# duckdb-faiss-ext/duckdb-faiss-ext

Hardware: AMD Instinct MI355X
Metric: queries/sec, FlatL2 d=128 N=10000000 nq=10000 k=10 (higher is better)
Workload: dtype f32 results (bf16 matrix-pipe coarse filter with a proven bound + exact f32 re-scoring of the candidates); 1 GPU; Flat L2 d=128 N=10000000 nq=10000 k=10; queries_per_call=10000, replicas=1, exchange=none

## Files before the change

duckdb-faiss-ext_amd/csrc/flat_collect.hip:

```cpp
#include "flat_collect.h"

#include <algorithm>
#include <climits>
#include <cmath>
#include <cstring>
#include <type_traits>

#include <rocprim/device/device_radix_sort.hpp>
#include <rocprim/device/device_segmented_radix_sort.hpp>

namespace mvs {

__global__ __launch_bounds__(256) void collect_colsum_kernel(const float *__restrict__ src, long long nrows, int dp,
                                                            int interleaved, float *__restrict__ sum) {
	const int g8 = dp / 8, rl = threadIdx.x / g8, c8 = threadIdx.x % g8, nrl = 256 / g8;
	float acc[8] = {0.f, 0.f, 0.f, 0.f, 0.f, 0.f, 0.f, 0.f};
	const long long r0 = (long long)blockIdx.x * 1024;
	__shared__ float red[256 * 8];
	const bool idle = rl >= nrl;
	for (long long r = r0 + rl; !idle && r < r0 + 1024 && r < nrows; r += nrl) {
		const float4 s0 = *(const float4 *)(src + (size_t)r * dp + c8 * 8);
		const float4 s1 = *(const float4 *)(src + (size_t)r * dp + c8 * 8 + 4);
		float v[8];
		if (!interleaved) {
// ... 470 lines not shown
				}
			}
		}
		part[which][r] = acc;
	}
	__syncthreads();
	if (tid < 64) {
		const long long q = q0 + tid;
		if (q < nq) {
			const float xn = part[0][tid], xnc = part[1][tid], mun = part[2][tid], dq2 = part[3][tid];
			qn[q] = xn;
			const float yn = __uint_as_float(max_norm_bits[2]), ync = __uint_as_float(max_norm_bits[8]);
			const float dyc = __uint_as_float(I8 ? i8_bits[0] : max_norm_bits[12]);
			const double u = 5.9604644775390625e-08, infl = 1.0001;
			const double S = sqrt((double)xn * infl) * sqrt((double)yn * infl);
			const double Sc = sqrt((double)xnc * infl) * sqrt((double)ync * infl);
			const double MY = sqrt((double)mun * infl) * sqrt((double)yn * infl);
			const double al = IS_L2 ? 2.0 : 1.0;
			const double bmax = IS_L2 ? (double)ync : MY;
			const double rnd_worst = al * (0.0078125 + 1.52587890625e-05) * Sc;
			const double ndq = sqrt((double)dq2 * infl), ndy = sqrt((double)dyc * infl);
			const double rnd_actual = ndq * sqrt((double)ync * infl) + (al * sqrt((double)xnc * infl) + ndq) * ndy;
			const double rnd = I8 ? rnd_actual
			                      : (bound_mode == 0 ? rnd_worst : (rnd_actual < rnd_worst || !(rnd_actual == rnd_actual) ? rnd_actual : rnd_worst));
			const double es = I8 ? rnd + 0.5 * (double)i8_unit
			                     : rnd + 1.25 * ((double)d / 16.0) * CL_MFMA_UNITS * u * ((1.0 + 0.0079) * al * Sc + bmax);
			double E;
			if (IS_L2)
				E = es + 4.0 * u * ((double)xnc + ync) + (double)d * u * ync + 2.0 * d * u * S + 4.0 * u * ((double)xn + yn) +
				    2.0 * ((double)d + 8.0) * u * ((double)xn + yn);
			else
				E = es + 4.0 * u * Sc + 2.0 * u * MY + (double)d * u * MY + (double)d * u * S;
			float r = (float)(2.0 * E * (1.0 + 0.0009765625) + 8.0 * u * (Sc + MY + (double)xnc + ync) + 1e-30);
			const bool ok = isfinite(xn) && isfinite(yn) && isfinite(ync) && isfinite(mun) && isfinite(dq2) && isfinite(dyc) && isfinite(r) && r < 1e30f;
			if (!ok) {
				r = __uint_as_float(0x7fc00000u);
				fail_q[atomicAdd(fail_cnt, 1)] = (int)q;
			}
			e2[q] = r;
		} else if (q < nq_e2) {
			e2[q] = __uint_as_float(0x7fc00000u);
		}
	}
	const float alpha = IS_L2 ? 2.0f : 1.0f;
	if (I8) {
		i32x4n *qf8 = (i32x4n *)qf;
		for (int i = tid; i < 4 * 2 * 64; i += 256) {
			const int lane = i & 63, kb = (i >> 6) & 1, qb = i >> 7;
			const int r = qb * 16 + (lane & 15);
			if (q0 + qb * 16 >= nq_frag)
				continue;
			i32x4n w = {0, 0, 0, 0};
#pragma unroll
			for (int e = 0; e < 16; ++e) {
				const int kk = kb * 64 + 16 * (lane >> 4) + e;
				const int qv = (q0 + r < nq && kk < d) ? cl_i8_q(alpha * (xs[r][kk] - ms[kk]), inv_sa) : 0;
				w[e >> 2] |= (int)((unsigned)(qv & 255) << (8 * (e & 3)));
			}
			qf8[((q0 / 16 + qb) * 2 + kb) * 64 + lane] = w;
		}
	}
	for (int i = tid; i < 4 * 4 * 64 && !I8; i += 256) {
		const int lane = i & 63, kb = (i >> 6) & 3, qb = i >> 8;
		const int r = qb * 16 + (lane & 15);
		if (q0 + qb * 16 >= nq_frag)
			continue;
		bf16x8 hi;
#pragma unroll
		for (int e = 0; e < 8; ++e) {
			const int kk = kb * 32 + 8 * (lane >> 4) + e;
			hi[e] = (__bf16)((q0 + r < nq && kk < d) ? alpha * (xs[r][kk] - ms[kk]) : 0.f);
		}
		qf[((q0 / 16 + qb) * 4 + kb) * 64 + lane] = hi;
	}
	const unsigned neutral = ~f2key(-FLT_MAX);
	for (int i = tid; i < 64 * stride; i += 256) {
		const long long q = q0 + i / stride;
		if (q < nq)
			gslot[q * stride + (i % stride)] = neutral;
	}
	if (tid < 64 && q0 + tid < nq) {
		ctl_seg[q0 + tid] = 0;
		ctl_seg[nq + q0 + tid] = 0;
	}
	if (blockIdx.x == 0 && tid < 64)
		ctl_hdr[tid] = 0;
}
void launch_collect_query_prep(int metric, const float *d_x, int64_t nq, int d, const float *d_mu, const unsigned *d_max_norm_bits,
                               void *d_qf, float *d_qn, float *d_e2, int *d_fail_cnt, int *d_fail_q, unsigned *d_gslot, int stride,
                               int *d_ctl_hdr, int *d_ctl_seg, hipStream_t st, const unsigned *d_i8_bits, float i8_sa, float i8_unit) {
	if (nq <= 0)
		return;
	const long long nq_frag = (nq + CL_QBLOCK - 1) / CL_QBLOCK * CL_QBLOCK, nq_e2 = (nq + 255) / 256 * 256;
	const dim3 grid((unsigned)(nq_frag / 64));
	const bool i8 = i8_unit > 0.f;
	auto kern = metric == METRIC_L2 ? (i8 ? collect_query_prep_kernel<true, true> : collect_query_prep_kernel<true>)
	                                : (i8 ? collect_query_prep_kernel<false, true> : collect_query_prep_kernel<false>);
	hipLaunchKernelGGL(kern, grid, dim3(256), 0, st, d_x, (long long)nq, d, d_mu, d_max_norm_bits, (bf16x8 *)d_qf, nq_frag, d_qn, d_e2, nq_e2,
	                   d_fail_cnt, d_fail_q, tune().cl_bound_mode, d_gslot, stride, d_ctl_hdr, d_ctl_seg, d_i8_bits, i8_sa, i8_unit);
	MVS_HIP(hipGetLastError());
}

typedef float f32x4acc __attribute__((ext_vector_type(4)));
template <int KCH, bool IS_L2, bool COLLECT, bool SEL = false, int NC = 16, bool I8 = false>
__global__ __launch_bounds__(256, I8 ? 3 : 2) void flat_bf16_collect_kernel(const CollectArgs a) {
	constexpr int DP = KCH * 16;
	constexpr int KB = I8 ? DP / 64 : DP / 32;
	constexpr int PITCH = I8 ? DP : DP * 2;
	constexpr int C = PITCH / 16;
	constexpr int TILE_BYTES = CL_BN * PITCH;
	constexpr int SUB = cl_sub(I8);
	constexpr int STAGE_ROWS = SUB * CL_BN;
	constexpr int STAGE_BYTES = SUB * TILE_BYTES;
	constexpr int NDMA = STAGE_BYTES / 1024;
	constexpr int DMA_PER_WAVE = NDMA / 4;
	constexpr int QCAP = cl_qcap(I8);
	static_assert(C == (I8 ? 8 : 16) && KB == (I8 ? 2 : 4) && NDMA % 4 == 0 && STAGE_ROWS % 64 == 0, "d = 128 geometry");
	typedef typename std::conditional<I8, i32x4n, bf16x8>::type frag_t;
	typedef typename std::conditional<I8, i32x4n, f32x4acc>::type acc_t;
	typedef typename std::conditional<I8, i32x2n, f32x2n>::type bnd_t;
	typedef typename std::conditional<I8, int, float>::type val_t;
	const float unit = a.i8_unit;

	extern __shared__ __attribute__((aligned(16))) float smem[];
	char *tbuf = (char *)smem;
	float *nbuf = (float *)(tbuf + 2 * STAGE_BYTES);
	unsigned long long *qbuf = (unsigned long long *)(nbuf + 2 * STAGE_ROWS);
	float *cqtab = (float *)(qbuf + QCAP);
	unsigned *qctl = (unsigned *)(cqtab + CL_QBLOCK);
	float *qval = (float *)(qctl + 16);
	float *cqstage = qval + QCAP;

	const int tid = threadIdx.x, lane = tid & 63;
	const int wave = __builtin_amdgcn_readfirstlane(tid >> 6);
	const int hq = lane >> 4, c = lane & 15;
	int split, qb;
	if (a.xcd_map) {
		const int xcd = blockIdx.x & 7, idx = blockIdx.x >> 3;
		split = (idx / a.nqb) * 8 + xcd;
		qb = idx % a.nqb;
	} else {
		split = blockIdx.x / a.nqb;
		qb = blockIdx.x % a.nqb;
	}
	const long long r_begin = a.row_first + (long long)split * a.split_rows;
	long long r_end = r_begin + a.split_rows;
	if (r_end > a.n)
		r_end = a.n;
	const int ntiles = r_end > r_begin ? (int)((r_end - r_begin + STAGE_ROWS - 1) / STAGE_ROWS) : 0;
	if (tid == 0)
		qctl[7] = 0u;

	const int qw = qb * CL_QBLOCK + wave * 128;

	frag_t bq[8][KB];
	{
		const frag_t *qsrc = (const frag_t *)a.qf;
#pragma unroll
		for (int cb = 0; cb < 8; ++cb) {
			const size_t qblk16 = (size_t)qb * (CL_QBLOCK / 16) + wave * 8 + cb;
#pragma unroll
			for (int kb = 0; kb < KB; ++kb)
				bq[cb][kb] = qsrc[(qblk16 * KB + kb) * 64 + lane];
		}
	}

	unsigned dma_off;
	{
		const int rr = I8 ? 8 * wave + (lane >> 3) : 4 * wave + (lane >> 4);
		dma_off = (unsigned)(rr * PITCH + (((lane & (C - 1)) ^ (rr & (C - 1))) * 16));
	}
	auto dma_issue = [&](int u, int i) {
		const char *base = (const char *)a.yb + (size_t)(r_begin + (long long)u * STAGE_ROWS) * PITCH + (size_t)i * 4096;
		__builtin_amdgcn_global_load_lds((glb_f32c *)(base + dma_off),
		                                 (lds_f32c *)(smem + ((u & 1) * STAGE_BYTES + (i * 4 + wave) * 1024) / 4), 16, 0, 0);
	};
	auto dma_norms = [&](int u) {
		const float *base = a.yn + (r_begin + (long long)u * STAGE_ROWS);
#pragma unroll
		for (int j = 0; j < STAGE_ROWS / 64; ++j)
			__builtin_amdgcn_global_load_lds((glb_f32c *)(base + 64 * j + lane),
			                                 (lds_f32c *)(smem + (2 * STAGE_BYTES) / 4 + (u & 1) * STAGE_ROWS + 64 * j), 4, 0, 0);
	};
	const bool use_tab = a.pbnd != nullptr;
	const bool frozen = use_tab && (a.flags & CL_FROZEN) != 0;
	constexpr int tab_shift = I8 ? 1 : 2;
	constexpr int duty_mask = (!COLLECT ? 3 : (NC > 32 ? 255 : 63)) >> (I8 ? 1 : 0);
	const int duty_phase = split * 13 + 5;
	bool tab_pending = false;
	const float inv_unit = I8 ? 1.0f / unit : 0.f;
	auto dma_bounds = [&]() {
		const float *base = a.pbnd + (size_t)qb * CL_QBLOCK + wave * 128;
		float *dst = (I8 ? cqstage : cqtab) + wave * 128;
		__builtin_amdgcn_global_load_lds((glb_f32c *)(base + lane), (lds_f32c *)dst, 4, 0, 16 );
		__builtin_amdgcn_global_load_lds((glb_f32c *)(base + 64 + lane), (lds_f32c *)(dst + 64), 4, 0, 16);
		tab_pending = I8;
	};
	auto tab_cvt = [&]() {
		if (!I8 || !tab_pending)
			return;
		tab_pending = false;
		const float p0 = cqstage[wave * 128 + lane], p1 = cqstage[wave * 128 + 64 + lane];
		((int *)cqtab)[wave * 128 + lane] = cl_i8_thr(p0, inv_unit);
		((int *)cqtab)[wave * 128 + 64 + lane] = cl_i8_thr(p1, inv_unit);
	};
	if (ntiles > 0) {
#pragma unroll
		for (int i = 0; i < DMA_PER_WAVE; ++i)
			dma_issue(0, i);
		dma_norms(0);
		if (use_tab)
			dma_bounds();
	}
	__syncthreads();
	tab_cvt();

	const unsigned rbase = (unsigned)(c * PITCH) | (unsigned)(((hq ^ c) & (C - 1)) * 16);
	constexpr int WQCAP = QCAP / 4;
	const unsigned qcnt_lds = (unsigned)(uintptr_t)((__attribute__((address_space(3))) unsigned *)qctl);
	const unsigned qbuf_lds = (unsigned)(uintptr_t)((__attribute__((address_space(3))) unsigned long long *)qbuf) + (unsigned)(wave * WQCAP * 8);
	const unsigned qval_lds = (unsigned)(uintptr_t)((__attribute__((address_space(3))) float *)qval) + (unsigned)(wave * WQCAP * 4);
	const unsigned cq_lds = (unsigned)(uintptr_t)((__attribute__((address_space(3))) float *)cqtab) + (unsigned)((wave * 64 + c) * 8);

	int ovf = 0;
	int wfill = 0, wpub = 0;
	auto publish = [&]() __attribute__((always_inline)) {
		const unsigned n = (unsigned)wfill < (unsigned)WQCAP ? (unsigned)wfill : (unsigned)WQCAP;
		for (unsigned e = (unsigned)wpub + lane; e < n && !frozen; e += 64) {
			unsigned long long ent;
			float v;
			asm volatile("ds_read_b64 %0, %2\n\tds_read_b32 %1, %3\n\ts_waitcnt lgkmcnt(0)"
			             : "=&v"(ent), "=&v"(v)
			             : "v"(qbuf_lds + 8u * e), "v"(qval_lds + 4u * e)
			             : "memory");
			const unsigned row = (unsigned)ent;
			typedef __attribute__((address_space(1))) unsigned *GU;
			__hip_atomic_fetch_min((GU)(a.gslot + (size_t)(unsigned)(ent >> 32) * NC) + (row & (unsigned)(NC - 1)), skey(v), __ATOMIC_RELAXED,
			                       __HIP_MEMORY_SCOPE_AGENT);
		}
		wpub = (int)n;
	};
	auto wdrain = [&]() __attribute__((always_inline)) {
		publish();
		const unsigned n = (unsigned)wpub;
		wfill = 0;
		wpub = 0;
		if (!COLLECT || n == 0u)
			return;
		unsigned long long base = 0ull;
		if (lane == 0) {
			const unsigned long long n64 = n;
			typedef __attribute__((address_space(1))) unsigned long long *GUL;
			asm volatile("global_atomic_add_x2 %0, %1, %2, off sc0\n\ts_waitcnt vmcnt(0)"
			             : "=&v"(base)
			             : "v"((GUL)a.stream_cnt), "v"(n64)
			             : "memory");
		}
		const unsigned blo = (unsigned)__builtin_amdgcn_readfirstlane((int)(unsigned)base);
		const unsigned bhi = (unsigned)__builtin_amdgcn_readfirstlane((int)(unsigned)(base >> 32));
		base = ((unsigned long long)bhi << 32) | blo;
		for (unsigned e = lane; e < n; e += 64) {
			unsigned long long ent;
			float v;
			asm volatile("ds_read_b64 %0, %2\n\tds_read_b32 %1, %3\n\ts_waitcnt lgkmcnt(0)"
			             : "=&v"(ent), "=&v"(v)
			             : "v"(qbuf_lds + 8u * e), "v"(qval_lds + 4u * e)
			             : "memory");
			if ((long long)(base + e) < a.stream_cap) {
				typedef __attribute__((address_space(1))) unsigned long long *GUL;
				*((GUL)a.stream + (base + e)) = ent;
				if (a.stream_s)
					a.stream_s[base + e] = v;
			}
		}
		ovf |= (long long)(base + n) >= a.stream_cap ? 1 : 0;
	};
	auto rare = [&](const acc_t (&sv)[2], int rb, int t, bool any_t, bnd_t cqv, long long row0, int nvalid, unsigned rowbits) {
		if (__builtin_expect(__builtin_amdgcn_ballot_w64(any_t) == 0ull, 1))
			return;
		int qo = qw;
		MVS_OPAQUE_VGPR(qo);
		unsigned m0 = 0u, m1 = 0u;
		if (any_t) {
#pragma unroll
			for (int r = 0; r < 4; ++r) {
				const bool in = 16 * rb + 4 * hq + r < nvalid;
				m0 |= (in && sv[0][r] >= cqv[0]) ? 1u << r : 0u;
				m1 |= (in && sv[1][r] >= cqv[1]) ? 1u << r : 0u;
			}
			if (SEL) {
				const unsigned rbits = (rowbits >> (16 * rb + 4 * hq)) & 15u;
				m0 &= rbits;
				m1 &= rbits;
			}
		}
		unsigned m = m0 | (m1 << 4);
		while (__builtin_amdgcn_ballot_w64(m != 0u) != 0ull) {
			const bool has = m != 0u;
			const int j8 = has ? __builtin_ctz(m) : 0;
			m &= m - 1u;
			const int i = j8 >> 2, j = j8 & 3;
			const val_t s0 = i ? sv[1][0] : sv[0][0], s1 = i ? sv[1][1] : sv[0][1], s2 = i ? sv[1][2] : sv[0][2], s3 = i ? sv[1][3] : sv[0][3];
			const val_t lo = (j & 1) ? s1 : s0;
			const val_t hi = (j & 1) ? s3 : s2;
			const float v = I8 ? (float)((j & 2) ? hi : lo) * unit : (float)((j & 2) ? hi : lo);
			const unsigned row = (unsigned)(row0 + 16 * rb + 4 * hq + j);
			const unsigned q = (unsigned)(qo + 32 * t + 16 * i + c);
			if (!(COLLECT && ovf) && __builtin_expect(wfill + (int)__builtin_popcountll(__builtin_amdgcn_ballot_w64(has)) > WQCAP, 0))
				wdrain();
			const bool counting = COLLECT && ovf;
			const unsigned long long act = __builtin_amdgcn_ballot_w64(has && !counting);
			const unsigned pos = (unsigned)wfill + __builtin_amdgcn_mbcnt_hi((unsigned)(act >> 32), __builtin_amdgcn_mbcnt_lo((unsigned)act, 0u));
			wfill = __builtin_amdgcn_readfirstlane(wfill + (int)__builtin_popcountll(act));
			if (has) {
				const unsigned long long ent = ((unsigned long long)q << 32) | row;
				if (__builtin_expect(!counting, 1)) {
					asm volatile("ds_write_b64 %0, %1\n\tds_write_b32 %2, %3" ::"v"(qbuf_lds + 8u * pos), "v"(ent), "v"(qval_lds + 4u * pos), "v"(v) : "memory");
				} else {
					typedef __attribute__((address_space(1))) unsigned *GU;
					__hip_atomic_fetch_min((GU)(a.gslot + (size_t)q * NC) + (row & (unsigned)(NC - 1)), skey(v), __ATOMIC_RELAXED,
					                       __HIP_MEMORY_SCOPE_AGENT);
					const unsigned one = 1u;
					asm volatile("ds_add_u32 %0, %1" ::"v"(qcnt_lds + 28u), "v"(one) : "memory");
				}
			}
		}
	};

	for (int u = 0; u < ntiles; ++u) {
		const int period = u < 4 ? 1 : (u < 32 ? 8 : (u < 256 ? 32 : 128));
		const bool full = !frozen && (use_tab ? ((u + duty_phase) & duty_mask) == 0 : (u % period) == 0);
		if (use_tab && !full && u > 0 && (u & ((1 << tab_shift) - 1)) == 0)
			dma_bounds();
		if (full) {
			publish();
			int qo = qw;
			MVS_OPAQUE_VGPR(qo);
			f32x2n v = {0.f, 0.f};
#pragma unroll 1
			for (int i = 0; i < 2; ++i) {
				const int q = qo + 32 * hq + 16 * i + c;
				const int qc = q < a.nq ? q : 0;
				const float e2v = __builtin_nontemporal_load(a.e2 + qc);
				constexpr int SUBN = NC > 32 ? 32 : NC, NSUB = NC / SUBN;
				const int rank = NSUB == 1 ? a.nclass - 1 : (a.nclass + NSUB - 1) / NSUB - 1;
				unsigned kth = 0u;
#pragma unroll 1
				for (int sb = 0; sb < NSUB; ++sb) {
				const unsigned long long *src = (const unsigned long long *)(a.gslot + (size_t)qc * NC + sb * SUBN);
				unsigned long long w[SUBN / 2];
#pragma unroll
				for (int j = 0; j < SUBN / 2; ++j)
					w[j] = __hip_atomic_load(src + j, __ATOMIC_RELAXED, __HIP_MEMORY_SCOPE_AGENT);
#pragma unroll
				for (int j = 0; j < SUBN / 2; ++j)
					asm volatile("" : "+v"(w[j]));
				unsigned key[SUBN];
#pragma unroll
				for (int j = 0; j < SUBN / 2; ++j) {
					key[2 * j] = (unsigned)w[j];
					key[2 * j + 1] = (unsigned)(w[j] >> 32);
				}
#pragma unroll
				for (int kbit = 2; kbit <= SUBN; kbit <<= 1)
#pragma unroll
					for (int jb = kbit >> 1; jb > 0; jb >>= 1)
#pragma unroll
						for (int x0 = 0; x0 < SUBN; ++x0) {
							const int x1 = x0 ^ jb;
							if (x1 > x0) {
								const unsigned lo = key[x0] < key[x1] ? key[x0] : key[x1];
								const unsigned hi = key[x0] < key[x1] ? key[x1] : key[x0];
								const bool asc = (x0 & kbit) == 0;
								key[x0] = asc ? lo : hi;
								key[x1] = asc ? hi : lo;
							}
						}
				unsigned ks = key[0];
#pragma unroll
				for (int j = 1; j < SUBN; ++j)
					ks = (rank == j) ? key[j] : ks;
				kth = ks > kth ? ks : kth;
				}
				const unsigned neutral = skey(-FLT_MAX);
				const float B = skey2f(kth < neutral ? kth : neutral);
				const float bv = q < a.nq ? B - e2v : __uint_as_float(0x7fc00000u);
				v[0] = i == 0 ? bv : v[0];
				v[1] = i == 1 ? bv : v[1];
			}
			if (I8) {
				const i32x2n vi = {cl_i8_thr(v[0], inv_unit), cl_i8_thr(v[1], inv_unit)};
				*(i32x2n *)(cqtab + (wave * 64 + hq * 16 + c) * 2) = vi;
			} else {
				*(f32x2n *)(cqtab + (wave * 64 + hq * 16 + c) * 2) = v;
			}
			if (use_tab) {
				unsigned long long bits;
				__builtin_memcpy(&bits, &v, 8);
				__hip_atomic_store((unsigned long long *)(a.pbnd + (size_t)qb * CL_QBLOCK + (wave * 64 + hq * 16 + c) * 2), bits, __ATOMIC_RELAXED,
				                   __HIP_MEMORY_SCOPE_AGENT);
			}
		}
#pragma unroll 1
		for (int sub = 0; sub < SUB; ++sub) {
		frag_t A[KB][2];
		acc_t Y[2];
		{
			const unsigned nb_lds = (unsigned)(uintptr_t)((lds_f32c *)(nbuf + (u & 1) * STAGE_ROWS + sub * CL_BN + 4 * hq));
			asm volatile("ds_read_b128 %0, %2\n\tds_read_b128 %1, %2 offset:64" : "=&v"(Y[0]), "=&v"(Y[1]) : "v"(nb_lds) : "memory");
			const unsigned ab =
			    (unsigned)(uintptr_t)((lds_f32c *)(smem + ((u & 1) * STAGE_BYTES + sub * TILE_BYTES) / 4)) + rbase;
#pragma unroll
			for (int kb = 0; kb < KB; ++kb) {
				asm volatile("ds_read_b128 %0, %1" : "=v"(A[kb][0]) : "v"(ab ^ (unsigned)(kb * 64)) : "memory");
				if (I8)
					asm volatile("ds_read_b128 %0, %1 offset:2048" : "=v"(A[kb][1]) : "v"(ab ^ (unsigned)(kb * 64)) : "memory");
				else
					asm volatile("ds_read_b128 %0, %1 offset:4096" : "=v"(A[kb][1]) : "v"(ab ^ (unsigned)(kb * 64)) : "memory");
			}
		}
		if (sub == 0) {
#pragma unroll
			for (int i = 0; i < DMA_PER_WAVE; ++i)
				dma_issue(u + 1, i);
			dma_norms(u + 1);
		}
		const long long row0 = r_begin + ((long long)u * SUB + sub) * CL_BN;
		const int nvalid = (int)((r_end - row0) < CL_BN ? (r_end - row0) : CL_BN);
		unsigned rowbits = 0xFFFFFFFFu;
		if (SEL) {
			typedef __attribute__((address_space(4))) const unsigned cuint;
			rowbits = *((cuint *)a.rowmask + (row0 >> 5));
		}

		acc_t acc[2][2];
		bnd_t cqv[2];
		const val_t lowest = I8 ? (val_t)INT_MIN : (val_t)-INFINITY;
		val_t mx0 = lowest, mx1 = lowest;
		auto vmax = [](val_t x, val_t y) {
			if constexpr (I8)
				return x > y ? x : y;
			else
				return __builtin_fmaxf(x, y);
		};
		auto fold = [&](acc_t &p, int rb, int i) {
			(void)rb;
			if (i == 0)
				mx0 = vmax(vmax(vmax(vmax(mx0, p[0]), p[1]), p[2]), p[3]);
			else
				mx1 = vmax(vmax(vmax(vmax(mx1, p[0]), p[1]), p[2]), p[3]);
		};
		auto any_of = [&](bnd_t cqp) {
			const bool r = (mx0 >= cqp[0]) || (mx1 >= cqp[1]);
			mx0 = lowest;
			mx1 = lowest;
			return r;
		};
#pragma unroll
		for (int t = 0; t < 4; ++t) {
			asm volatile("ds_read_b64 %0, %1" : "=v"(cqv[t & 1]) : "v"(cq_lds + (unsigned)(t * 128)) : "memory");
#pragma unroll
			for (int rb = 0; rb < 2; ++rb) {
				const int prb = rb ^ 1, pt = rb == 0 ? t - 1 : t;
#pragma unroll
				for (int kb = 0; kb < KB; ++kb) {
					if constexpr (I8) {
						if (t == 0) {
							if (rb == 0 && kb == 0)
								asm volatile("s_waitcnt lgkmcnt(4)" : "+v"(A[0][0]), "+v"(Y[0]), "+v"(Y[1]));
							else if (rb == 0 && kb == 1)
								asm volatile("s_waitcnt lgkmcnt(2)" : "+v"(A[1][0]));
							else if (rb == 1 && kb == 0)
								asm volatile("s_waitcnt lgkmcnt(0)" : "+v"(A[0][1]), "+v"(A[1][1]), "+v"(cqv[0]));
						}
					} else if (t == 0) {
						if (rb == 0 && kb == 0)
							asm volatile("s_waitcnt lgkmcnt(8)" : "+v"(A[0][0]), "+v"(Y[0]), "+v"(Y[1]));
						else if (rb == 0 && kb == 1)
							asm volatile("s_waitcnt lgkmcnt(6)" : "+v"(A[1][0]));
						else if (rb == 0 && kb == 2)
							asm volatile("s_waitcnt lgkmcnt(4)" : "+v"(A[2][0]));
						else if (rb == 0 && kb == 3)
							asm volatile("s_waitcnt lgkmcnt(2)" : "+v"(A[3][0]));
						else if (rb == 1 && kb == 0)
							asm volatile("s_waitcnt lgkmcnt(0)" : "+v"(A[0][1]), "+v"(A[1][1]), "+v"(A[2][1]), "+v"(A[3][1]), "+v"(cqv[0]));
					}
#pragma unroll
					for (int i = 0; i < 2; ++i) {
						if constexpr (I8)
							acc[rb][i] = __builtin_amdgcn_mfma_i32_16x16x64_i8(A[kb][rb], bq[2 * t + i][kb], kb == 0 ? Y[rb] : acc[rb][i], 0, 0, 0);
						else if (kb == 0)
							acc[rb][i] = __builtin_amdgcn_mfma_f32_16x16x32_bf16(A[kb][rb], bq[2 * t + i][kb], Y[rb], 0, 0, 0);
						else
							acc[rb][i] = __builtin_amdgcn_mfma_f32_16x16x32_bf16(A[kb][rb], bq[2 * t + i][kb], acc[rb][i], 0, 0, 0);
					}
					if (pt >= 0 && kb < 2)
						fold(acc[prb][kb], prb, kb);
					__builtin_amdgcn_sched_barrier(0);
				}
				if (pt >= 0) {
					if (rb == 0)
						asm volatile("s_waitcnt lgkmcnt(0)" : "+v"(cqv[0]), "+v"(cqv[1]));
					rare(acc[prb], prb, pt, any_of(cqv[pt & 1]), cqv[pt & 1], row0, nvalid, rowbits);
				}
			}
		}
		{
			fold(acc[1][0], 1, 0);
			fold(acc[1][1], 1, 1);
			rare(acc[1], 1, 3, any_of(cqv[1]), cqv[1], row0, nvalid, rowbits);
		}
		}
		__syncthreads();
		tab_cvt();
		constexpr int FLUSH_EVERY = I8 ? CL_FLUSH_EVERY / 2 : CL_FLUSH_EVERY;
		static_assert(FLUSH_EVERY >= 1, "queue cadence");
		if ((u % FLUSH_EVERY) == FLUSH_EVERY - 1 || u == ntiles - 1) {
			if (wfill >= WQCAP / 2 || u == ntiles - 1)
				wdrain();
			else
				publish();
		}
	}
	if (COLLECT) {
		__syncthreads();
		if (tid == 0 && qctl[7] != 0u)
			atomicAdd(a.stream_cnt, (unsigned long long)qctl[7]);
	}
}

constexpr size_t cl_lds_bytes(bool i8) {
	return (size_t)2 * cl_sub(i8) * CL_BN * 128 * (i8 ? 1 : 2) + (size_t)2 * cl_sub(i8) * CL_BN * 4 + (size_t)cl_qcap(i8) * 8 + (size_t)CL_QBLOCK * 4 + 64 +
	       (size_t)cl_qcap(i8) * 4 + (i8 ? (size_t)CL_QBLOCK * 4 : 0);
}
static_assert(3 * cl_lds_bytes(true) <= 160 * 1024 && 2 * cl_lds_bytes(false) <= 160 * 1024, "LDS per workgroup of the d <= 128 scan");
static size_t collect_lds_bytes(const FlatGeom &g, bool i8) {
	(void)g;
	return cl_lds_bytes(i8);
}

bool collect_supported(const FlatGeom &g) {
	return collect_store_dims(g.d) > 0;
}

__device__ __forceinline__ bool cl_sel_member(const SelectorDev &s, long long id) {
	if (s.kind == MVS_SEL_BITMAP) {
		const unsigned long long u = (unsigned long long)id;
		if ((u >> 3) >= (unsigned long long)s.nbytes)
			return false;
		return (s.bitmap[u >> 3] >> (u & 7)) & 1;
	}
	if (s.kind == MVS_SEL_BATCH) {
		long long lo = 0, hi = s.nids;
		while (lo < hi) {
			const long long mid = (lo + hi) >> 1;
			if (s.sorted_ids[mid] < id)
				lo = mid + 1;
			else
				hi = mid;
		}
		return lo < s.nids && s.sorted_ids[lo] == id;
	}
	return true;
}
__global__ __launch_bounds__(256) void collect_rowmask_kernel(SelectorDev sel, const long long *__restrict__ idmap, long long n,
                                                             long long nwords, unsigned long long *__restrict__ mask) {
	const long long row = (long long)blockIdx.x * blockDim.x + threadIdx.x;
	bool ok = false;
	if (row < n)
		ok = cl_sel_member(sel, idmap ? idmap[row] : row);
	const unsigned long long b = __builtin_amdgcn_ballot_w64(ok);
	if ((threadIdx.x & 63) == 0 && (row >> 6) < nwords)
		mask[row >> 6] = b;
}
size_t collect_rowmask_bytes(int64_t n) {
	return (size_t)((n + 63) / 64 + 64) * 8;
}
void launch_collect_rowmask(SelectorDev sel, const int64_t *d_idmap, int64_t n, unsigned long long *d_mask, hipStream_t st) {
	const long long nwords = (long long)(collect_rowmask_bytes(n) / 8);
	const long long rows = nwords * 64;
	hipLaunchKernelGGL(collect_rowmask_kernel, dim3((unsigned)((rows + 255) / 256)), dim3(256), 0, st, sel,
	                   (const long long *)d_idmap, (long long)n, nwords, d_mask);
	MVS_HIP(hipGetLastError());
}


int flat_mfma_slot_stride(int64_t k);
__global__ void init_gslot_kernel(unsigned *g, long long total, int stride, int k, int is_l2);

template <int NC>
__global__ void collect_bound_table_kernel(const unsigned *__restrict__ gslot, const float *__restrict__ e2, int nclass, int nq,
                                           long long total, float *__restrict__ pbnd) {
	const long long j = (long long)blockIdx.x * blockDim.x + threadIdx.x;
	if (j >= total)
		return;
	const int o = (int)(j & 127), w = (int)((j >> 7) & 3);
	const long long qb = j >> 9;
	const int i = o & 1, c = (o >> 1) & 15, hq = o >> 5;
	const long long q = qb * CL_QBLOCK + w * 128 + 32 * hq + 16 * i + c;
	float bv = __uint_as_float(0x7fc00000u);
	if (q < nq) {
		constexpr int SUBN = NC > 32 ? 32 : NC, NSUB = NC / SUBN;
		const int rank = NSUB == 1 ? nclass - 1 : (nclass + NSUB - 1) / NSUB - 1;
		unsigned kth = 0u;
		for (int sb = 0; sb < NSUB; ++sb) {
			unsigned key[SUBN];
#pragma unroll
			for (int t = 0; t < SUBN; ++t)
				key[t] = gslot[(size_t)q * NC + sb * SUBN + t];
			unsigned ks = 0xffffffffu;
#pragma unroll
			for (int t = 0; t < SUBN; ++t) {
				int less = 0, leq = 0;
#pragma unroll
				for (int s2 = 0; s2 < SUBN; ++s2) {
					less += key[s2] < key[t];
					leq += key[s2] <= key[t];
				}
				if (less <= rank && rank < leq)
					ks = key[t];
			}
			kth = ks > kth ? ks : kth;
		}
		const unsigned neutral = skey(-FLT_MAX);
		const float B = skey2f(kth < neutral ? kth : neutral);
		bv = B - e2[q];
	}
	pbnd[j] = bv;
}
static void launch_collect_bound_table(const CollectArgs &a, int nqb, hipStream_t st) {
	if (!a.pbnd)
		return;
	const long long total = (long long)nqb * CL_QBLOCK;
	const dim3 grid((unsigned)((total + 255) / 256));
	if (a.slot_stride == 128)
		hipLaunchKernelGGL(collect_bound_table_kernel<128>, grid, dim3(256), 0, st, (const unsigned *)a.gslot, a.e2, a.nclass, a.nq, total, a.pbnd);
	else if (a.slot_stride == 32)
		hipLaunchKernelGGL(collect_bound_table_kernel<32>, grid, dim3(256), 0, st, (const unsigned *)a.gslot, a.e2, a.nclass, a.nq, total, a.pbnd);
	else
		hipLaunchKernelGGL(collect_bound_table_kernel<16>, grid, dim3(256), 0, st, (const unsigned *)a.gslot, a.e2, a.nclass, a.nq, total, a.pbnd);
	MVS_HIP(hipGetLastError());
}
size_t collect_bound_table_bytes(int64_t nq) {
	return (size_t)((nq + CL_QBLOCK - 1) / CL_QBLOCK) * CL_QBLOCK * sizeof(float) + 1024;
}

template <bool COLLECT>
static void launch_collect_range(const FlatGeom &g, int metric, CollectArgs a, int64_t row_first, int64_t row_end,
                                 int64_t nsplit_want, int64_t nq, hipStream_t st, int *grid_out, int *nsplit_out) {
	const int nqb = (int)((nq + CL_QBLOCK - 1) / CL_QBLOCK);
	if (!tune().cl_tab && !(a.flags & CL_FROZEN))
		a.pbnd = nullptr;
	if (!(a.flags & CL_FROZEN))
		launch_collect_bound_table(a, nqb, st);
	const bool i8 = a.i8_unit > 0.f;
	const int64_t stage_rows = cl_sub(i8) * CL_BN;
	const int64_t ntiles = (row_end - row_first + stage_rows - 1) / stage_rows;
	const int64_t nsplit = std::max<int64_t>(1, std::min<int64_t>(nsplit_want, ntiles));
	a.xcd_map = (nsplit >= 8 && nsplit % 8 == 0) ? 1 : 0;
	a.row_first = row_first;
	a.n = row_end;
	a.split_rows = (ntiles + nsplit - 1) / nsplit * stage_rows;
	a.nqb = nqb;
	a.nsplit = (int)nsplit;
	const int grid = nqb * (int)nsplit;
	const size_t lds = collect_lds_bytes(g, i8);
#define MVS_CL_GO(L2, SEL_, NC_)                                                                                        \
	{                                                                                                                  \
		auto kern = i8 ? flat_bf16_collect_kernel<8, L2, COLLECT, SEL_, NC_, true> : flat_bf16_collect_kernel<8, L2, COLLECT, SEL_, NC_>; \
		ensure_dynamic_lds((const void *)kern, lds);                                                                   \
		hipLaunchKernelGGL(kern, dim3(grid), dim3(256), lds, st, a);                                                   \
	}
	if (a.slot_stride == 32 || a.slot_stride == 128) {
#define MVS_CL_NC32(L2, SEL_)                                                                                           \
	{                                                                                                                  \
		if (a.slot_stride == 128)                                                                                      \
			MVS_CL_GO(L2, SEL_, 128)                                                                                   \
		else                                                                                                           \
			MVS_CL_GO(L2, SEL_, 32)                                                                                    \
	}
		if (a.rowmask && metric == METRIC_L2)
			MVS_CL_NC32(true, true)
// ... 1060 lines not shown
```

Before: 993,300 queries/s.

## Pipeline int8 coarse-filter sub-tiles with double-buffered LDS fragments and deferred rescans

Adds a dedicated I8 path in the collect kernel. It fully unrolls the sub-tile loop and double-buffers A fragments and norms, prefetching the next sub-tile during the last t-step. Per-tile hit checks are recorded as wave-ballot bit flags, and the rare candidate handling runs afterwards by recomputing the flagged MFMA blocks. Waves whose queries lie beyond nq skip compute and only issue the DMA. This aims to hide LDS latency and take branchy rare() calls out of the MFMA stream, at the cost of more VGPRs and recomputation when hits occur. The workload is described as a bf16 pipeline, so this I8 path may not run.

```diff
diff --git a/duckdb-faiss-ext_amd/csrc/flat_collect.hip b/duckdb-faiss-ext_amd/csrc/flat_collect.hip
--- a/duckdb-faiss-ext_amd/csrc/flat_collect.hip
+++ b/duckdb-faiss-ext_amd/csrc/flat_collect.hip
@@ -646,6 +646,7 @@
 		qctl[7] = 0u;
 
 	const int qw = qb * CL_QBLOCK + wave * 128;
+	const bool dead = I8 && qw >= a.nq;
 
 	frag_t bq[8][KB];
 	{
@@ -895,6 +896,146 @@
 				                   __HIP_MEMORY_SCOPE_AGENT);
 			}
 		}
+		if constexpr (I8) {
+		if (dead) {
+#pragma unroll
+			for (int i = 0; i < DMA_PER_WAVE; ++i)
+				dma_issue(u + 1, i);
+			dma_norms(u + 1);
+		} else {
+		const unsigned st_lds = (unsigned)(uintptr_t)((lds_f32c *)(smem + ((u & 1) * STAGE_BYTES) / 4)) + rbase;
+		const unsigned sn_lds = (unsigned)(uintptr_t)((lds_f32c *)(nbuf + (u & 1) * STAGE_ROWS + 4 * hq));
+		unsigned flags = 0u;
+		frag_t A[2][KB][2];
+		acc_t Y[2];
+		auto fetch_beta = [&](int rb, int sub) __attribute__((always_inline)) {
+			asm volatile("ds_read_b128 %0, %1" : "=v"(Y[rb]) : "v"(sn_lds + (unsigned)(sub * CL_BN * 4 + rb * 64)) : "memory");
+		};
+		auto fetch = [&](int s, int sub) __attribute__((always_inline)) {
+#pragma unroll
+			for (int kb = 0; kb < KB; ++kb) {
+				const unsigned ab = (st_lds + (unsigned)(sub * TILE_BYTES)) ^ (unsigned)(kb * 64);
+				asm volatile("ds_read_b128 %0, %1" : "=v"(A[s][kb][0]) : "v"(ab) : "memory");
+				asm volatile("ds_read_b128 %0, %1 offset:2048" : "=v"(A[s][kb][1]) : "v"(ab) : "memory");
+			}
+		};
+#pragma unroll
+		for (int sub = 0; sub < SUB; ++sub) {
+			const int s = sub & 1;
+			const bool fetched = sub > 0;
+			const bool fetch_next = sub + 1 < SUB;
+			if (!fetched) {
+				fetch_beta(0, sub);
+				fetch_beta(1, sub);
+				fetch(s, sub);
+			}
+			if (sub == 0) {
+#pragma unroll
+				for (int i = 0; i < DMA_PER_WAVE; ++i)
+					dma_issue(u + 1, i);
+				dma_norms(u + 1);
+			}
+			acc_t acc[2][2];
+			bnd_t cqv[2];
+			int mx0 = INT_MIN, mx1 = INT_MIN;
+			auto imax = [](int x, int y) { return x > y ? x : y; };
+			auto fold = [&](acc_t &p, int i) {
+				if (i == 0)
+					mx0 = imax(imax(imax(imax(mx0, p[0]), p[1]), p[2]), p[3]);
+				else
+					mx1 = imax(imax(imax(imax(mx1, p[0]), p[1]), p[2]), p[3]);
+			};
+			auto hit = [&](int pt, int prb) __attribute__((always_inline)) {
+				const bool any0 = mx0 >= cqv[pt & 1][0], any1 = mx1 >= cqv[pt & 1][1];
+				mx0 = INT_MIN;
+				mx1 = INT_MIN;
+				flags |= (__builtin_amdgcn_ballot_w64(any0) | __builtin_amdgcn_ballot_w64(any1)) != 0ull ? (1u << (2 * pt + prb)) << (8 * sub) : 0u;
+			};
+#pragma unroll
+			for (int t = 0; t < 4; ++t) {
+				asm volatile("ds_read_b64 %0, %1" : "=v"(cqv[t & 1]) : "v"(cq_lds + (unsigned)(t * 128)) : "memory");
+				if (t == 3 && fetch_next)
+					fetch(s ^ 1, sub + 1);
+#pragma unroll
+				for (int rb = 0; rb < 2; ++rb) {
+					const int prb = rb ^ 1, pt = rb == 0 ? t - 1 : t;
+#pragma unroll
+					for (int kb = 0; kb < KB; ++kb) {
+						if (t == 0 && fetched) {
+							if (rb == 0 && kb == 0)
+								asm volatile("s_waitcnt lgkmcnt(2)" : "+v"(Y[0]), "+v"(A[s][0][0]), "+v"(A[s][0][1]), "+v"(A[s][1][0]), "+v"(A[s][1][1]));
+							else if (rb == 1 && kb == 0)
+								asm volatile("s_waitcnt lgkmcnt(0)" : "+v"(Y[1]), "+v"(cqv[0]));
+						} else if (t == 0) {
+							if (rb == 0 && kb == 0)
+								asm volatile("s_waitcnt lgkmcnt(4)" : "+v"(A[s][0][0]), "+v"(Y[0]), "+v"(Y[1]));
+							else if (rb == 0 && kb == 1)
+								asm volatile("s_waitcnt lgkmcnt(2)" : "+v"(A[s][1][0]));
+							else if (rb == 1 && kb == 0)
+								asm volatile("s_waitcnt lgkmcnt(0)" : "+v"(A[s][0][1]), "+v"(A[s][1][1]), "+v"(cqv[0]));
+						}
+#pragma unroll
+						for (int i = 0; i < 2; ++i)
+							acc[rb][i] = __builtin_amdgcn_mfma_i32_16x16x64_i8(A[s][kb][rb], bq[2 * t + i][kb], kb == 0 ? Y[rb] : acc[rb][i], 0, 0, 0);
+						if (pt >= 0) {
+							__builtin_amdgcn_sched_barrier(0);
+							fold(acc[prb][kb], kb);
+						}
+						__builtin_amdgcn_sched_barrier(0);
+						if (t == 3 && fetch_next && kb == 0)
+							fetch_beta(rb, sub + 1);
+					}
+					if (pt >= 0) {
+						if (rb == 0) {
+							if (t == 3 && fetch_next)
+								asm volatile("s_waitcnt lgkmcnt(5)" : "+v"(cqv[0]), "+v"(cqv[1]));
+							else
+								asm volatile("s_waitcnt lgkmcnt(0)" : "+v"(cqv[0]), "+v"(cqv[1]));
+						}
+						hit(pt, prb);
+					}
+				}
+			}
+			fold(acc[1][0], 0);
+			fold(acc[1][1], 1);
+			hit(3, 1);
+		}
+		if (__builtin_expect(flags != 0u, 0)) {
+			unsigned fl = flags;
+			do {
+				const int b = __builtin_ctz(fl);
+				fl &= fl - 1u;
+				const int sub = b >> 3, t = (b >> 1) & 3, rb = b & 1;
+				frag_t Ar[KB];
+				acc_t Yr, sv[2];
+				bnd_t cq;
+				const unsigned ab = st_lds + (unsigned)(sub * TILE_BYTES);
+				asm volatile("ds_read_b128 %0, %4\n\tds_read_b128 %1, %5\n\tds_read_b128 %2, %6\n\tds_read_b64 %3, %7\n\ts_waitcnt lgkmcnt(0)"
+				             : "=&v"(Yr), "=&v"(Ar[0]), "=&v"(Ar[1]), "=&v"(cq)
+				             : "v"(sn_lds + (unsigned)(sub * CL_BN * 4 + rb * 64)), "v"(ab + (unsigned)(rb * 2048)), "v"((ab ^ 64u) + (unsigned)(rb * 2048)),
+				               "v"(cq_lds + (unsigned)(t * 128))
+				             : "memory");
+#pragma unroll
+				for (int tt = 0; tt < 4; ++tt)
+					if (t == tt) {
+#pragma unroll
+						for (int i = 0; i < 2; ++i) {
+							sv[i] = __builtin_amdgcn_mfma_i32_16x16x64_i8(Ar[0], bq[2 * tt + i][0], Yr, 0, 0, 0);
+							sv[i] = __builtin_amdgcn_mfma_i32_16x16x64_i8(Ar[1], bq[2 * tt + i][1], sv[i], 0, 0, 0);
+						}
+					}
+				const long long row0 = r_begin + ((long long)u * SUB + sub) * CL_BN;
+				const int nvalid = (int)((r_end - row0) < CL_BN ? (r_end - row0) : CL_BN);
+				unsigned rowbits = 0xFFFFFFFFu;
+				if (SEL) {
+					typedef __attribute__((address_space(4))) const unsigned cuint;
+					rowbits = *((cuint *)a.rowmask + (row0 >> 5));
+				}
+				rare(sv, rb, t, true, cq, row0, nvalid, rowbits);
+			} while (fl != 0u);
+		}
+		}
+		} else {
 #pragma unroll 1
 		for (int sub = 0; sub < SUB; ++sub) {
 		frag_t A[KB][2];
@@ -907,10 +1048,7 @@
 #pragma unroll
 			for (int kb = 0; kb < KB; ++kb) {
 				asm volatile("ds_read_b128 %0, %1" : "=v"(A[kb][0]) : "v"(ab ^ (unsigned)(kb * 64)) : "memory");
-				if (I8)
-					asm volatile("ds_read_b128 %0, %1 offset:2048" : "=v"(A[kb][1]) : "v"(ab ^ (unsigned)(kb * 64)) : "memory");
-				else
-					asm volatile("ds_read_b128 %0, %1 offset:4096" : "=v"(A[kb][1]) : "v"(ab ^ (unsigned)(kb * 64)) : "memory");
+				asm volatile("ds_read_b128 %0, %1 offset:4096" : "=v"(A[kb][1]) : "v"(ab ^ (unsigned)(kb * 64)) : "memory");
 			}
 		}
 		if (sub == 0) {
@@ -929,14 +1067,9 @@
 
 		acc_t acc[2][2];
 		bnd_t cqv[2];
-		const val_t lowest = I8 ? (val_t)INT_MIN : (val_t)-INFINITY;
-		val_t mx0 = lowest, mx1 = lowest;
-		auto vmax = [](val_t x, val_t y) {
-			if constexpr (I8)
-				return x > y ? x : y;
-			else
-				return __builtin_fmaxf(x, y);
-		};
+		const float lowest = -INFINITY;
+		float mx0 = lowest, mx1 = lowest;
+		auto vmax = [](float x, float y) { return __builtin_fmaxf(x, y); };
 		auto fold = [&](acc_t &p, int rb, int i) {
 			(void)rb;
 			if (i == 0)
@@ -958,16 +1091,7 @@
 				const int prb = rb ^ 1, pt = rb == 0 ? t - 1 : t;
 #pragma unroll
 				for (int kb = 0; kb < KB; ++kb) {
-					if constexpr (I8) {
-						if (t == 0) {
-							if (rb == 0 && kb == 0)
-								asm volatile("s_waitcnt lgkmcnt(4)" : "+v"(A[0][0]), "+v"(Y[0]), "+v"(Y[1]));
-							else if (rb == 0 && kb == 1)
-								asm volatile("s_waitcnt lgkmcnt(2)" : "+v"(A[1][0]));
-							else if (rb == 1 && kb == 0)
-								asm volatile("s_waitcnt lgkmcnt(0)" : "+v"(A[0][1]), "+v"(A[1][1]), "+v"(cqv[0]));
-						}
-					} else if (t == 0) {
+					if (t == 0) {
 						if (rb == 0 && kb == 0)
 							asm volatile("s_waitcnt lgkmcnt(8)" : "+v"(A[0][0]), "+v"(Y[0]), "+v"(Y[1]));
 						else if (rb == 0 && kb == 1)
@@ -981,9 +1105,7 @@
 					}
 #pragma unroll
 					for (int i = 0; i < 2; ++i) {
-						if constexpr (I8)
-							acc[rb][i] = __builtin_amdgcn_mfma_i32_16x16x64_i8(A[kb][rb], bq[2 * t + i][kb], kb == 0 ? Y[rb] : acc[rb][i], 0, 0, 0);
-						else if (kb == 0)
+						if (kb == 0)
 							acc[rb][i] = __builtin_amdgcn_mfma_f32_16x16x32_bf16(A[kb][rb], bq[2 * t + i][kb], Y[rb], 0, 0, 0);
 						else
 							acc[rb][i] = __builtin_amdgcn_mfma_f32_16x16x32_bf16(A[kb][rb], bq[2 * t + i][kb], acc[rb][i], 0, 0, 0);
@@ -1003,6 +1125,7 @@
 			fold(acc[1][0], 1, 0);
 			fold(acc[1][1], 1, 1);
 			rare(acc[1], 1, 3, any_of(cqv[1]), cqv[1], row0, nvalid, rowbits);
+		}
 		}
 		}
 		__syncthreads();
```

After: 1.008 million queries/s, median of 6. +1.5%, better.

## Prefetch next sub-tile fragments and scalarize DMA addressing in int8 scan path

Applied to the files above, without the earlier changes.

In the int8 coarse-scan path, the LDS reads for the next sub-tile's fragments and norms are issued during the current sub-tile's final MFMA steps instead of at the top of each iteration. The wait counts are adjusted to match. DMA base addresses are made wave-uniform with readfirstlane so addressing stays scalar. Norm loads are split across waves and the bounds load is merged into a single 16-byte load per even wave. This aims to hide LDS latency and cut VALU address work, at the cost of more fragile hand-tuned waitcnt ordering.

```diff
diff --git a/duckdb-faiss-ext_amd/csrc/flat_collect.hip b/duckdb-faiss-ext_amd/csrc/flat_collect.hip
--- a/duckdb-faiss-ext_amd/csrc/flat_collect.hip
+++ b/duckdb-faiss-ext_amd/csrc/flat_collect.hip
@@ -664,17 +664,39 @@
 		const int rr = I8 ? 8 * wave + (lane >> 3) : 4 * wave + (lane >> 4);
 		dma_off = (unsigned)(rr * PITCH + (((lane & (C - 1)) ^ (rr & (C - 1))) * 16));
 	}
+	auto sbase = [](const void *p) {
+		const unsigned long long v = (unsigned long long)(uintptr_t)p;
+		const unsigned lo = (unsigned)__builtin_amdgcn_readfirstlane((int)(unsigned)v);
+		const unsigned hi = (unsigned)__builtin_amdgcn_readfirstlane((int)(unsigned)(v >> 32));
+		return (const char *)(uintptr_t)(((unsigned long long)hi << 32) | lo);
+	};
+	unsigned lane4 = (unsigned)lane * 4u;
 	auto dma_issue = [&](int u, int i) {
 		const char *base = (const char *)a.yb + (size_t)(r_begin + (long long)u * STAGE_ROWS) * PITCH + (size_t)i * 4096;
-		__builtin_amdgcn_global_load_lds((glb_f32c *)(base + dma_off),
-		                                 (lds_f32c *)(smem + ((u & 1) * STAGE_BYTES + (i * 4 + wave) * 1024) / 4), 16, 0, 0);
+		if constexpr (I8) {
+			MVS_OPAQUE_VGPR(dma_off);
+			__builtin_amdgcn_global_load_lds((glb_f32c *)(sbase(base) + dma_off),
+			                                 (lds_f32c *)(smem + ((u & 1) * STAGE_BYTES + (i * 4 + wave) * 1024) / 4), 16, 0, 0);
+		} else {
+			__builtin_amdgcn_global_load_lds((glb_f32c *)(base + dma_off),
+			                                 (lds_f32c *)(smem + ((u & 1) * STAGE_BYTES + (i * 4 + wave) * 1024) / 4), 16, 0, 0);
+		}
 	};
 	auto dma_norms = [&](int u) {
 		const float *base = a.yn + (r_begin + (long long)u * STAGE_ROWS);
-#pragma unroll
-		for (int j = 0; j < STAGE_ROWS / 64; ++j)
-			__builtin_amdgcn_global_load_lds((glb_f32c *)(base + 64 * j + lane),
-			                                 (lds_f32c *)(smem + (2 * STAGE_BYTES) / 4 + (u & 1) * STAGE_ROWS + 64 * j), 4, 0, 0);
+		if constexpr (I8) {
+			const int j = (wave - u) & 3;
+			if (j < STAGE_ROWS / 64) {
+				MVS_OPAQUE_VGPR(lane4);
+				__builtin_amdgcn_global_load_lds((glb_f32c *)(sbase(base + 64 * j) + lane4),
+				                                 (lds_f32c *)(smem + (2 * STAGE_BYTES) / 4 + (u & 1) * STAGE_ROWS + 64 * j), 4, 0, 0);
+			}
+		} else {
+#pragma unroll
+			for (int j = 0; j < STAGE_ROWS / 64; ++j)
+				__builtin_amdgcn_global_load_lds((glb_f32c *)(base + 64 * j + lane),
+				                                 (lds_f32c *)(smem + (2 * STAGE_BYTES) / 4 + (u & 1) * STAGE_ROWS + 64 * j), 4, 0, 0);
+		}
 	};
 	const bool use_tab = a.pbnd != nullptr;
 	const bool frozen = use_tab && (a.flags & CL_FROZEN) != 0;
@@ -686,8 +708,16 @@
 	auto dma_bounds = [&]() {
 		const float *base = a.pbnd + (size_t)qb * CL_QBLOCK + wave * 128;
 		float *dst = (I8 ? cqstage : cqtab) + wave * 128;
-		__builtin_amdgcn_global_load_lds((glb_f32c *)(base + lane), (lds_f32c *)dst, 4, 0, 16 );
-		__builtin_amdgcn_global_load_lds((glb_f32c *)(base + 64 + lane), (lds_f32c *)(dst + 64), 4, 0, 16);
+		if constexpr (I8) {
+			if ((wave & 1) == 0) {
+				unsigned lane16 = lane4 * 4u;
+				MVS_OPAQUE_VGPR(lane16);
+				__builtin_amdgcn_global_load_lds((glb_f32c *)(sbase(base) + lane16), (lds_f32c *)dst, 16, 0, 16 );
+			}
+		} else {
+			__builtin_amdgcn_global_load_lds((glb_f32c *)(base + lane), (lds_f32c *)dst, 4, 0, 16 );
+			__builtin_amdgcn_global_load_lds((glb_f32c *)(base + 64 + lane), (lds_f32c *)(dst + 64), 4, 0, 16);
+		}
 		tab_pending = I8;
 	};
 	auto tab_cvt = [&]() {
@@ -895,115 +925,136 @@
 				                   __HIP_MEMORY_SCOPE_AGENT);
 			}
 		}
-#pragma unroll 1
-		for (int sub = 0; sub < SUB; ++sub) {
 		frag_t A[KB][2];
 		acc_t Y[2];
-		{
-			const unsigned nb_lds = (unsigned)(uintptr_t)((lds_f32c *)(nbuf + (u & 1) * STAGE_ROWS + sub * CL_BN + 4 * hq));
-			asm volatile("ds_read_b128 %0, %2\n\tds_read_b128 %1, %2 offset:64" : "=&v"(Y[0]), "=&v"(Y[1]) : "v"(nb_lds) : "memory");
-			const unsigned ab =
-			    (unsigned)(uintptr_t)((lds_f32c *)(smem + ((u & 1) * STAGE_BYTES + sub * TILE_BYTES) / 4)) + rbase;
-#pragma unroll
-			for (int kb = 0; kb < KB; ++kb) {
-				asm volatile("ds_read_b128 %0, %1" : "=v"(A[kb][0]) : "v"(ab ^ (unsigned)(kb * 64)) : "memory");
-				if (I8)
-					asm volatile("ds_read_b128 %0, %1 offset:2048" : "=v"(A[kb][1]) : "v"(ab ^ (unsigned)(kb * 64)) : "memory");
-				else
-					asm volatile("ds_read_b128 %0, %1 offset:4096" : "=v"(A[kb][1]) : "v"(ab ^ (unsigned)(kb * 64)) : "memory");
-			}
-		}
-		if (sub == 0) {
+#define MVS_FRAG_FETCH(NB, AB, RB, YOFF, AOFF)                                                                                       \
+	do {                                                                                                                            \
+		asm volatile("ds_read_b128 %0, %1 offset:" #YOFF : "=v"(Y[RB]) : "v"(NB) : "memory");                                        \
+		asm volatile("ds_read_b128 %0, %1 offset:" #AOFF : "=v"(A[0][RB]) : "v"(AB) : "memory");                                     \
+		asm volatile("ds_read_b128 %0, %1 offset:" #AOFF : "=v"(A[1][RB]) : "v"((AB) ^ 64u) : "memory");                             \
+	} while (0)
+		static_assert(!I8 || (KB == 2 && CL_BN * 4 == 128 && TILE_BYTES == 4096), "the offsets of MVS_FRAG_FETCH");
+		if constexpr (I8) {
+			const unsigned nb_lds = (unsigned)(uintptr_t)((lds_f32c *)(nbuf + (u & 1) * STAGE_ROWS + 4 * hq));
+			const unsigned ab = (unsigned)(uintptr_t)((lds_f32c *)(smem + ((u & 1) * STAGE_BYTES) / 4)) + rbase;
+			MVS_FRAG_FETCH(nb_lds, ab, 0, 0, 0);
+			MVS_FRAG_FETCH(nb_lds, ab, 1, 64, 2048);
 #pragma unroll
 			for (int i = 0; i < DMA_PER_WAVE; ++i)
 				dma_issue(u + 1, i);
 			dma_norms(u + 1);
 		}
-		const long long row0 = r_begin + ((long long)u * SUB + sub) * CL_BN;
-		const int nvalid = (int)((r_end - row0) < CL_BN ? (r_end - row0) : CL_BN);
-		unsigned rowbits = 0xFFFFFFFFu;
-		if (SEL) {
-			typedef __attribute__((address_space(4))) const unsigned cuint;
-			rowbits = *((cuint *)a.rowmask + (row0 >> 5));
-		}
-
-		acc_t acc[2][2];
-		bnd_t cqv[2];
-		const val_t lowest = I8 ? (val_t)INT_MIN : (val_t)-INFINITY;
-		val_t mx0 = lowest, mx1 = lowest;
-		auto vmax = [](val_t x, val_t y) {
-			if constexpr (I8)
-				return x > y ? x : y;
-			else
-				return __builtin_fmaxf(x, y);
-		};
-		auto fold = [&](acc_t &p, int rb, int i) {
-			(void)rb;
-			if (i == 0)
-				mx0 = vmax(vmax(vmax(vmax(mx0, p[0]), p[1]), p[2]), p[3]);
-			else
-				mx1 = vmax(vmax(vmax(vmax(mx1, p[0]), p[1]), p[2]), p[3]);
-		};
-		auto any_of = [&](bnd_t cqp) {
-			const bool r = (mx0 >= cqp[0]) || (mx1 >= cqp[1]);
-			mx0 = lowest;
-			mx1 = lowest;
-			return r;
-		};
-#pragma unroll
-		for (int t = 0; t < 4; ++t) {
-			asm volatile("ds_read_b64 %0, %1" : "=v"(cqv[t & 1]) : "v"(cq_lds + (unsigned)(t * 128)) : "memory");
-#pragma unroll
-			for (int rb = 0; rb < 2; ++rb) {
-				const int prb = rb ^ 1, pt = rb == 0 ? t - 1 : t;
+#pragma unroll 1
+		for (int sub = 0; sub < SUB; ++sub) {
+			const unsigned nb_lds = (unsigned)(uintptr_t)((lds_f32c *)(nbuf + (u & 1) * STAGE_ROWS + sub * CL_BN + 4 * hq));
+			const unsigned ab = (unsigned)(uintptr_t)((lds_f32c *)(smem + ((u & 1) * STAGE_BYTES + sub * TILE_BYTES) / 4)) + rbase;
+			if constexpr (!I8) {
+				asm volatile("ds_read_b128 %0, %2\n\tds_read_b128 %1, %2 offset:64" : "=&v"(Y[0]), "=&v"(Y[1]) : "v"(nb_lds) : "memory");
 #pragma unroll
 				for (int kb = 0; kb < KB; ++kb) {
+					asm volatile("ds_read_b128 %0, %1" : "=v"(A[kb][0]) : "v"(ab ^ (unsigned)(kb * 64)) : "memory");
+					asm volatile("ds_read_b128 %0, %1 offset:4096" : "=v"(A[kb][1]) : "v"(ab ^ (unsigned)(kb * 64)) : "memory");
+				}
+				if (sub == 0) {
+#pragma unroll
+					for (int i = 0; i < DMA_PER_WAVE; ++i)
+						dma_issue(u + 1, i);
+					dma_norms(u + 1);
+				}
+			}
+			const long long row0 = r_begin + ((long long)u * SUB + sub) * CL_BN;
+			const int nvalid = (int)((r_end - row0) < CL_BN ? (r_end - row0) : CL_BN);
+			unsigned rowbits = 0xFFFFFFFFu;
+			if (SEL) {
+				typedef __attribute__((address_space(4))) const unsigned cuint;
+				rowbits = *((cuint *)a.rowmask + (row0 >> 5));
+			}
+
+			acc_t acc[2][2];
+			bnd_t cqv[2];
+			const val_t lowest = I8 ? (val_t)INT_MIN : (val_t)-INFINITY;
+			val_t mx0 = lowest, mx1 = lowest;
+			auto vmax = [](val_t x, val_t y) {
+				if constexpr (I8)
+					return x > y ? x : y;
+				else
+					return __builtin_fmaxf(x, y);
+			};
+			auto fold = [&](acc_t &p, int rb, int i) {
+				(void)rb;
+				if (i == 0)
+					mx0 = vmax(vmax(vmax(vmax(mx0, p[0]), p[1]), p[2]), p[3]);
+				else
+					mx1 = vmax(vmax(vmax(vmax(mx1, p[0]), p[1]), p[2]), p[3]);
+			};
+			auto any_of = [&](bnd_t cqp) {
+				const bool r = (mx0 >= cqp[0]) || (mx1 >= cqp[1]);
+				mx0 = lowest;
+				mx1 = lowest;
+				return r;
+			};
+#pragma unroll
+			for (int t = 0; t < 4; ++t) {
+				asm volatile("ds_read_b64 %0, %1" : "=v"(cqv[t & 1]) : "v"(cq_lds + (unsigned)(t * 128)) : "memory");
+#pragma unroll
+				for (int rb = 0; rb < 2; ++rb) {
+					const int prb = rb ^ 1, pt = rb == 0 ? t - 1 : t;
+#pragma unroll
+					for (int kb = 0; kb < KB; ++kb) {
+						if constexpr (I8) {
+							if (t == 0) {
+								if (rb == 0 && kb == 0)
+									asm volatile("s_waitcnt lgkmcnt(5)" : "+v"(A[0][0]), "+v"(Y[0]));
+								else if (rb == 0 && kb == 1)
+									asm volatile("s_waitcnt lgkmcnt(4)" : "+v"(A[1][0]));
+								else if (rb == 1 && kb == 0)
+									asm volatile("s_waitcnt lgkmcnt(0)" : "+v"(Y[1]), "+v"(A[0][1]), "+v"(A[1][1]), "+v"(cqv[0]));
+							}
+						} else if (t == 0) {
+							if (rb == 0 && kb == 0)
+								asm volatile("s_waitcnt lgkmcnt(8)" : "+v"(A[0][0]), "+v"(Y[0]), "+v"(Y[1]));
+							else if (rb == 0 && kb == 1)
+								asm volatile("s_waitcnt lgkmcnt(6)" : "+v"(A[1][0]));
+							else if (rb == 0 && kb == 2)
+								asm volatile("s_waitcnt lgkmcnt(4)" : "+v"(A[2][0]));
+							else if (rb == 0 && kb == 3)
+								asm volatile("s_waitcnt lgkmcnt(2)" : "+v"(A[3][0]));
+							else if (rb == 1 && kb == 0)
+								asm volatile("s_waitcnt lgkmcnt(0)" : "+v"(A[0][1]), "+v"(A[1][1]), "+v"(A[2][1]), "+v"(A[3][1]), "+v"(cqv[0]));
+						}
+#pragma unroll
+						for (int i = 0; i < 2; ++i) {
+							if constexpr (I8)
+								acc[rb][i] = __builtin_amdgcn_mfma_i32_16x16x64_i8(A[kb][rb], bq[2 * t + i][kb], kb == 0 ? Y[rb] : acc[rb][i], 0, 0, 0);
+							else if (kb == 0)
+								acc[rb][i] = __builtin_amdgcn_mfma_f32_16x16x32_bf16(A[kb][rb], bq[2 * t + i][kb], Y[rb], 0, 0, 0);
+							else
+								acc[rb][i] = __builtin_amdgcn_mfma_f32_16x16x32_bf16(A[kb][rb], bq[2 * t + i][kb], acc[rb][i], 0, 0, 0);
+						}
+						if (pt >= 0 && kb < 2)
+							fold(acc[prb][kb], prb, kb);
+						__builtin_amdgcn_sched_barrier(0);
+					}
 					if constexpr (I8) {
-						if (t == 0) {
-							if (rb == 0 && kb == 0)
-								asm volatile("s_waitcnt lgkmcnt(4)" : "+v"(A[0][0]), "+v"(Y[0]), "+v"(Y[1]));
-							else if (rb == 0 && kb == 1)
-								asm volatile("s_waitcnt lgkmcnt(2)" : "+v"(A[1][0]));
-							else if (rb == 1 && kb == 0)
-								asm volatile("s_waitcnt lgkmcnt(0)" : "+v"(A[0][1]), "+v"(A[1][1]), "+v"(cqv[0]));
+						if (t == 3 && rb == 1 && sub + 1 < SUB)
+							MVS_FRAG_FETCH(nb_lds, ab, 1, 192, 6144);
+					}
+					if (pt >= 0) {
+						if (rb == 0)
+							asm volatile("s_waitcnt lgkmcnt(0)" : "+v"(cqv[0]), "+v"(cqv[1]));
+						if constexpr (I8) {
+							if (t == 3 && rb == 0 && sub + 1 < SUB)
+								MVS_FRAG_FETCH(nb_lds, ab, 0, 128, 4096);
 						}
-					} else if (t == 0) {
-						if (rb == 0 && kb == 0)
-							asm volatile("s_waitcnt lgkmcnt(8)" : "+v"(A[0][0]), "+v"(Y[0]), "+v"(Y[1]));
-						else if (rb == 0 && kb == 1)
-							asm volatile("s_waitcnt lgkmcnt(6)" : "+v"(A[1][0]));
-						else if (rb == 0 && kb == 2)
-							asm volatile("s_waitcnt lgkmcnt(4)" : "+v"(A[2][0]));
-						else if (rb == 0 && kb == 3)
-							asm volatile("s_waitcnt lgkmcnt(2)" : "+v"(A[3][0]));
-						else if (rb == 1 && kb == 0)
-							asm volatile("s_waitcnt lgkmcnt(0)" : "+v"(A[0][1]), "+v"(A[1][1]), "+v"(A[2][1]), "+v"(A[3][1]), "+v"(cqv[0]));
+						rare(acc[prb], prb, pt, any_of(cqv[pt & 1]), cqv[pt & 1], row0, nvalid, rowbits);
 					}
-#pragma unroll
-					for (int i = 0; i < 2; ++i) {
-						if constexpr (I8)
-							acc[rb][i] = __builtin_amdgcn_mfma_i32_16x16x64_i8(A[kb][rb], bq[2 * t + i][kb], kb == 0 ? Y[rb] : acc[rb][i], 0, 0, 0);
-						else if (kb == 0)
-							acc[rb][i] = __builtin_amdgcn_mfma_f32_16x16x32_bf16(A[kb][rb], bq[2 * t + i][kb], Y[rb], 0, 0, 0);
-						else
-							acc[rb][i] = __builtin_amdgcn_mfma_f32_16x16x32_bf16(A[kb][rb], bq[2 * t + i][kb], acc[rb][i], 0, 0, 0);
-					}
-					if (pt >= 0 && kb < 2)
-						fold(acc[prb][kb], prb, kb);
-					__builtin_amdgcn_sched_barrier(0);
 				}
-				if (pt >= 0) {
-					if (rb == 0)
-						asm volatile("s_waitcnt lgkmcnt(0)" : "+v"(cqv[0]), "+v"(cqv[1]));
-					rare(acc[prb], prb, pt, any_of(cqv[pt & 1]), cqv[pt & 1], row0, nvalid, rowbits);
-				}
-			}
-		}
-		{
-			fold(acc[1][0], 1, 0);
-			fold(acc[1][1], 1, 1);
-			rare(acc[1], 1, 3, any_of(cqv[1]), cqv[1], row0, nvalid, rowbits);
-		}
+			}
+			{
+				fold(acc[1][0], 1, 0);
+				fold(acc[1][1], 1, 1);
+				rare(acc[1], 1, 3, any_of(cqv[1]), cqv[1], row0, nvalid, rowbits);
+			}
 		}
 		__syncthreads();
 		tab_cvt();
@@ -1022,6 +1073,7 @@
 			atomicAdd(a.stream_cnt, (unsigned long long)qctl[7]);
 	}
 }
+#undef MVS_FRAG_FETCH
 
 constexpr size_t cl_lds_bytes(bool i8) {
 	return (size_t)2 * cl_sub(i8) * CL_BN * 128 * (i8 ? 1 : 2) + (size_t)2 * cl_sub(i8) * CL_BN * 4 + (size_t)cl_qcap(i8) * 8 + (size_t)CL_QBLOCK * 4 + 64 +
```

New measurement: 1.025 million queries/s before, 1.042 million queries/s after (median of 6 runs). 1.6% higher.
